# arkworks-rs/gemini

Hardware: AMD Instinct MI355X
Metric: BLS12-381 G1 MSM throughput (higher is better)
Workload: dtype u32x12 Montgomery Fq (381-bit integer), u32x8 Fr; 1 GPU; 2^20 G1 MSM per GPU (BASELINE configs[1]: 2^20 G1 MSM on one MI355X); pairs_per_gpu=1048576

## Files before the change

gemini_amd/csrc/msm.hip:

```cpp
#include <algorithm>
#include <atomic>
#include <chrono>
#include <condition_variable>
#include <cstdlib>
#include <cstring>
#include <functional>
#include <sched.h>
#include <cstdio>
#include <thread>
#include <vector>

#include "ctx.hpp"
#include "g1.cuh"
#include "host_field.hpp"

namespace gm {

constexpr uint32_t KEY_INV = 0xffffffffu;
constexpr int XYZZ_BYTES = 192;
constexpr int AFF_BYTES = 96;

struct DigitIter {
  uint32_t s[8];
  uint32_t carry;
// ... 556 lines not shown
  }
}

struct FlatGeom {
  int c, W;
  int glv;
  uint32_t B;
  uint32_t K[8];
};
template <bool SCATTER>
__global__ __launch_bounds__(256) void k_digits_flat(const uint32_t* __restrict__ scalars, uint32_t n, int mont, FlatGeom fg,
                                                     uint32_t* __restrict__ counts_or_cursor, uint64_t* __restrict__ entries,
                                                     uint32_t* __restrict__ err) {
  const uint32_t i = blockIdx.x * blockDim.x + threadIdx.x;
  const int half = (int)blockIdx.y >= fg.W ? 1 : 0;
  const int w = (int)blockIdx.y - half * fg.W;
  const bool active = i < n;
  uint32_t key = KEY_INV;
  bool neg = false;
  if (active) {
    Fr v = fp_load<FrParams>(scalars + 8 * (size_t)i);
    if (mont) v = fp_from_mont<FrParams>(v);
    if (!SCATTER && blockIdx.y == 0 && (v.l[7] >> 31)) atomicOr(err, 1u);
    bool hneg = false;
#ifdef GM_EXPERIMENTS
    if (fg.glv) {
      const GlvHalves h = glv_split(v.l);
      hneg = h.neg[half];
#pragma unroll
      for (int l = 0; l < 8; l++) v.l[l] = l < 4 ? h.m[half][l] : 0u;
    }
#endif
    uint32_t t[9];
    uint32_t carry = 0;
#pragma unroll
    for (int l = 0; l < 8; l++) {
      uint32_t cy;
      t[l] = __builtin_addc(v.l[l], fg.K[l], carry, &cy);
      carry = cy;
    }
    t[8] = carry;
    const uint32_t bit = (uint32_t)(fg.c * w), lo = bit >> 5, sh = bit & 31u;
    uint64_t two = 0;
#pragma unroll
    for (int l = 0; l < 9; l++) {
      if ((uint32_t)l == lo) two |= (uint64_t)t[l];
      if ((uint32_t)l == lo + 1) two |= (uint64_t)t[l] << 32;
    }
    uint32_t u = (uint32_t)(two >> sh);
    int32_t d;
    if (w == fg.W - 1) {
      d = (int32_t)min(u, fg.B);
    } else {
      u &= (1u << fg.c) - 1u;
      d = (int32_t)u - (int32_t)(1u << (fg.c - 1));
    }
    if (d != 0) {
      key = (uint32_t)w * fg.B + ((uint32_t)(d < 0 ? -d : d) - 1u);
      neg = (d < 0) != hneg;
    }
  }
  const uint32_t pos = wave_atomic_inc(counts_or_cursor, key);
  if (SCATTER && key != KEY_INV)
    entries[pos] = ((uint64_t)key << 32) | ((uint64_t)(neg ? 1u : 0u) << 31) | (uint64_t)(i | ((uint32_t)half << ENTRY_HALF_SHIFT));
}

struct MultiGeom {
  int c, W, levels, step;
  uint32_t B;
  uint32_t K[8];
  uint32_t start[MULTI_MAX_LEVELS + 1];
  const uint32_t* scal[MULTI_MAX_LEVELS];
  long long base0[MULTI_MAX_LEVELS];
};
template <bool SCATTER>
__global__ __launch_bounds__(256) void k_digits_multi(MultiGeom mg, int mont, uint32_t* __restrict__ counts_or_cursor, uint64_t* __restrict__ entries,
                                                      uint32_t* __restrict__ err) {
  const uint32_t i = blockIdx.x * blockDim.x + threadIdx.x;
  const int w = (int)blockIdx.y;
  const bool active = i < mg.start[mg.levels];
  uint32_t key = KEY_INV, idx = 0;
  bool neg = false;
  if (active) {
    int l = 0;
    while (l + 1 < mg.levels && i >= mg.start[l + 1]) l++;
    const uint32_t il = i - mg.start[l];
    Fr v = fp_load<FrParams>(mg.scal[l] + 8 * (size_t)il);
    if (mont) v = fp_from_mont<FrParams>(v);
    if (!SCATTER && blockIdx.y == 0 && (v.l[7] >> 31)) atomicOr(err, 1u);
    uint32_t t[9];
    uint32_t carry = 0;
#pragma unroll
    for (int q = 0; q < 8; q++) {
      uint32_t cy;
      t[q] = __builtin_addc(v.l[q], mg.K[q], carry, &cy);
      carry = cy;
    }
    t[8] = carry;
    const uint32_t bit = (uint32_t)(mg.c * w), lo = bit >> 5, sh = bit & 31u;
    uint64_t two = 0;
#pragma unroll
    for (int q = 0; q < 9; q++) {
      if ((uint32_t)q == lo) two |= (uint64_t)t[q];
      if ((uint32_t)q == lo + 1) two |= (uint64_t)t[q] << 32;
    }
    uint32_t u = (uint32_t)(two >> sh);
    int32_t d;
    if (w == mg.W - 1) {
      d = (int32_t)min(u, mg.B);
    } else {
      u &= (1u << mg.c) - 1u;
      d = (int32_t)u - (int32_t)(1u << (mg.c - 1));
    }
    if (d != 0) {
      key = (uint32_t)(l * mg.W + w) * mg.B + ((uint32_t)(d < 0 ? -d : d) - 1u);
      neg = d < 0;
      idx = (uint32_t)(mg.base0[l] + (long long)mg.step * (long long)il);
    }
  }
  const uint32_t pos = wave_atomic_inc(counts_or_cursor, key);
  if (SCATTER && key != KEY_INV) entries[pos] = ((uint64_t)key << 32) | ((uint64_t)(neg ? 1u : 0u) << 31) | (uint64_t)idx;
}


__global__ __launch_bounds__(1024) void k_scan_small(const uint32_t* __restrict__ counts, uint32_t m, uint32_t* __restrict__ offsets,
                                                     uint32_t* __restrict__ cursor) {
  __shared__ uint32_t part[1024];
  const uint32_t tid = threadIdx.x;
  const uint32_t per = (m + 1023u) / 1024u;
  const uint32_t lo = min(tid * per, m), hi = min(lo + per, m);
  uint32_t s = 0;
  for (uint32_t k = lo; k < hi; k++) s += counts[k];
  part[tid] = s;
  __syncthreads();
  for (uint32_t d = 1; d < 1024; d <<= 1) {
    const uint32_t x = tid >= d ? part[tid - d] : 0;
    __syncthreads();
    part[tid] += x;
    __syncthreads();
  }
  uint32_t run = part[tid] - s;
  for (uint32_t k = lo; k < hi; k++) {
    const uint32_t c = counts[k];
    offsets[k] = run;
    cursor[k] = run;
    run += c;
  }
  if (tid == 1023) offsets[m] = part[1023];
}

#ifdef GM_ACC0_CYCLES
__device__ unsigned long long gm_acc0_dbg[4];
#endif
template <int WAVES>
__global__ __launch_bounds__(256) __attribute__((amdgpu_waves_per_eu(WAVES, WAVES))) void k_acc0(const uint64_t* __restrict__ entries,
                                              const uint32_t* __restrict__ total_ptr,
                                              const uint8_t* __restrict__ bases, long long first, long long step,
                                              long long tab_stride, uint32_t L, uint32_t* __restrict__ pk,
                                              uint8_t* __restrict__ pp, uint8_t* __restrict__ buckets, const uint8_t* __restrict__ phi,
                                              unsigned long long* __restrict__ clk) {
  __shared__ uint64_t ebuf[8][256];
  const uint32_t t = blockIdx.x * blockDim.x + threadIdx.x;
  const uint64_t clk_c0 = clock64(), clk_w0 = wall_clock64();
  const uint64_t total = *total_ptr;
  const uint64_t start = (uint64_t)t * L;
  uint32_t head_key = KEY_INV, tail_key = KEY_INV;
#ifdef GM_ACC0_CYCLES
  const uint64_t dbg_c0 = clock64(), dbg_w0 = wall_clock64();
#endif
  if (start < total) {
    const uint64_t end = min(start + (uint64_t)L, total);
    Acc30 acc;
    acc30_zero(acc);
    uint32_t cur = KEY_INV;
    bool first_run = true;
    for (uint64_t i = start; i < end; i++) {
      const uint32_t k8 = (uint32_t)(i - start) & 7u;
      if (k8 == 0) {
        const uint4* src = reinterpret_cast<const uint4*>(entries + i);
#pragma unroll
        for (int q = 0; q < 4; q++) {
          const uint4 v = src[q];
          ebuf[2 * q][threadIdx.x] = ((uint64_t)v.y << 32) | v.x;
          ebuf[2 * q + 1][threadIdx.x] = ((uint64_t)v.w << 32) | v.z;
        }
      }
      const uint64_t e = ebuf[k8][threadIdx.x];
      long long idx;
      if (tab_stride) {
        const uint32_t lo = (uint32_t)e & 0x7fffffffu;
        idx = (long long)(lo >> ENTRY_W_SHIFT) * tab_stride + first + step * (long long)(lo & ((1u << ENTRY_W_SHIFT) - 1u));
      } else {
        idx = first + step * (long long)(e & 0x3fffffffull);
      }
      const uint8_t* src = (phi != nullptr && ((e >> ENTRY_HALF_SHIFT) & 1ull)) ? phi : bases;
      const gm_u4v* bp = reinterpret_cast<const gm_u4v*>(src + (size_t)idx * AFF_BYTES);
      const gm_u4v x0 = bp[0], x1 = bp[1], x2 = bp[2], y0 = bp[3], y1 = bp[4], y2 = bp[5];
      const uint32_t key = (uint32_t)(e >> 32);
      if (key != cur) {
        if (cur != KEY_INV) {
          if (first_run) {
            head_key = cur;
            acc30_store(pp + (size_t)(2 * (size_t)t) * XYZZ30_BYTES, acc);
            first_run = false;
          } else {
            acc30_store(buckets + (size_t)cur * XYZZ30_BYTES, acc);
          }
        }
        cur = key;
        acc30_set_identity(acc);
      }
      const uint32_t nz = x0.x | x0.y | x0.z | x0.w | x1.x | x1.y | x1.z | x1.w | x2.x | x2.y | x2.z | x2.w | y0.x | y0.y | y0.z | y0.w |
                          y1.x | y1.y | y1.z | y1.w | y2.x | y2.y | y2.z | y2.w;
      if (nz == 0) continue;
      const uint32_t neg = (uint32_t)(e >> 31) & 1u;
      (void)g1_madd30_asm(acc, x0, x1, x2, y0, y1, y2, neg);
    }
    if (first_run) {
      head_key = cur;
      acc30_store(pp + (size_t)(2 * (size_t)t) * XYZZ30_BYTES, acc);
    } else {
      tail_key = cur;
      acc30_store(pp + (size_t)(2 * (size_t)t + 1) * XYZZ30_BYTES, acc);
    }
  }
  pk[2 * (size_t)t] = head_key;
  pk[2 * (size_t)t + 1] = tail_key;
  if (t == 0 && clk != nullptr) {
    clk[0] = (unsigned long long)(clock64() - clk_c0);
    clk[1] = (unsigned long long)(wall_clock64() - clk_w0);
  }
#ifdef GM_ACC0_CYCLES
  if ((threadIdx.x & 63) == 0) {
    atomicAdd(&gm_acc0_dbg[0], (unsigned long long)(clock64() - dbg_c0));
    atomicAdd(&gm_acc0_dbg[1], (unsigned long long)(wall_clock64() - dbg_w0));
    atomicAdd(&gm_acc0_dbg[2], 1ull);
  }
#endif
}

template <int WAVES>
__global__ __launch_bounds__(256) __attribute__((amdgpu_waves_per_eu(WAVES, WAVES))) void k_acc0_pf(const uint64_t* __restrict__ entries,
                                              const uint32_t* __restrict__ total_ptr,
                                              const uint8_t* __restrict__ bases, long long first, long long step,
                                              long long tab_stride, uint32_t L, uint32_t* __restrict__ pk,
                                              uint8_t* __restrict__ pp, uint8_t* __restrict__ buckets, const uint8_t* __restrict__ phi,
                                              unsigned long long* __restrict__ clk) {
  __shared__ uint64_t ebuf[8][256];
  const uint32_t t = blockIdx.x * blockDim.x + threadIdx.x;
  const uint64_t clk_c0 = clock64(), clk_w0 = wall_clock64();
  const uint64_t total = *total_ptr;
  const uint64_t start = (uint64_t)t * L;
  uint32_t head_key = KEY_INV, tail_key = KEY_INV;
  if (start < total) {
    const uint64_t end = min(start + (uint64_t)L, total);
    Acc30 acc;
    acc30_zero(acc);
    uint32_t cur = KEY_INV;
    bool first_run = true;
    auto entry_at = [&](uint64_t i) {
      const uint32_t k8 = (uint32_t)(i - start) & 7u;
      if (k8 == 0) {
        const uint4* src = reinterpret_cast<const uint4*>(entries + i);
#pragma unroll
        for (int q = 0; q < 4; q++) {
          const uint4 v = src[q];
          ebuf[2 * q][threadIdx.x] = ((uint64_t)v.y << 32) | v.x;
          ebuf[2 * q + 1][threadIdx.x] = ((uint64_t)v.w << 32) | v.z;
        }
      }
      return ebuf[k8][threadIdx.x];
    };
    auto base_of = [&](uint64_t e) {
      long long idx;
      if (tab_stride) {
        const uint32_t lo = (uint32_t)e & 0x7fffffffu;
        idx = (long long)(lo >> ENTRY_W_SHIFT) * tab_stride + first + step * (long long)(lo & ((1u << ENTRY_W_SHIFT) - 1u));
      } else {
        idx = first + step * (long long)(e & 0x3fffffffull);
      }
      const uint8_t* src = (phi != nullptr && ((e >> ENTRY_HALF_SHIFT) & 1ull)) ? phi : bases;
      return reinterpret_cast<const gm_u4v*>(src + (size_t)idx * AFF_BYTES);
    };
    uint64_t e = entry_at(start);
    const gm_u4v* bp = base_of(e);
    gm_u4v x0 = bp[0], x1 = bp[1], x2 = bp[2], y0 = bp[3], y1 = bp[4], y2 = bp[5];
    for (uint64_t i = start; i < end; i++) {
      uint64_t en = 0;
      gm_u4v n0 = x0, n1 = x1, n2 = x2, n3 = y0, n4 = y1, n5 = y2;
      if (i + 1 < end) {
        en = entry_at(i + 1);
        const gm_u4v* np = base_of(en);
        asm volatile(
            "global_load_dwordx4 %0, %6, off\n\t"
            "global_load_dwordx4 %1, %6, off offset:16\n\t"
            "global_load_dwordx4 %2, %6, off offset:32\n\t"
            "global_load_dwordx4 %3, %6, off offset:48\n\t"
            "global_load_dwordx4 %4, %6, off offset:64\n\t"
            "global_load_dwordx4 %5, %6, off offset:80"
            : "=&v"(n0), "=&v"(n1), "=&v"(n2), "=&v"(n3), "=&v"(n4), "=&v"(n5)
            : "v"(np));
      }
      const uint32_t key = (uint32_t)(e >> 32);
      if (key != cur) {
        if (cur != KEY_INV) {
          if (first_run) {
            head_key = cur;
            acc30_store(pp + (size_t)(2 * (size_t)t) * XYZZ30_BYTES, acc);
            first_run = false;
          } else {
            acc30_store(buckets + (size_t)cur * XYZZ30_BYTES, acc);
          }
        }
        cur = key;
        acc30_set_identity(acc);
      }
      const uint32_t nz = x0.x | x0.y | x0.z | x0.w | x1.x | x1.y | x1.z | x1.w | x2.x | x2.y | x2.z | x2.w | y0.x | y0.y | y0.z | y0.w |
                          y1.x | y1.y | y1.z | y1.w | y2.x | y2.y | y2.z | y2.w;
      if (nz != 0) {
        const uint32_t neg = (uint32_t)(e >> 31) & 1u;
        (void)g1_madd30_asm(acc, x0, x1, x2, y0, y1, y2, neg);
      }
      asm volatile("s_waitcnt vmcnt(0)" : "+v"(n0), "+v"(n1), "+v"(n2), "+v"(n3), "+v"(n4), "+v"(n5));
      e = en;
      x0 = n0; x1 = n1; x2 = n2; y0 = n3; y1 = n4; y2 = n5;
    }
    if (first_run) {
      head_key = cur;
      acc30_store(pp + (size_t)(2 * (size_t)t) * XYZZ30_BYTES, acc);
    } else {
      tail_key = cur;
      acc30_store(pp + (size_t)(2 * (size_t)t + 1) * XYZZ30_BYTES, acc);
    }
  }
  pk[2 * (size_t)t] = head_key;
  pk[2 * (size_t)t + 1] = tail_key;
  if (t == 0 && clk != nullptr) {
    clk[0] = (unsigned long long)(clock64() - clk_c0);
    clk[1] = (unsigned long long)(wall_clock64() - clk_w0);
  }
}

#ifdef GM_EXPERIMENTS
#include "msm_levels.inc"
#endif

__global__ __launch_bounds__(64) void k_merge(const uint32_t* __restrict__ keys_in, const uint8_t* __restrict__ pts_in,
                                              uint32_t E, uint32_t* __restrict__ keys_out,
                                              uint8_t* __restrict__ pts_out, uint8_t* __restrict__ buckets,
                                              int final_level) {
  __shared__ __attribute__((aligned(16))) uint8_t lds[128 * XYZZ30_BYTES];
  const int lane = threadIdx.x;
  const uint32_t wave = blockIdx.x;
  const uint32_t s0 = wave * 128u + 2u * lane;
  uint32_t hk = s0 < E ? keys_in[s0] : KEY_INV;
  uint32_t tk = s0 + 1 < E ? keys_in[s0 + 1] : KEY_INV;
  uint32_t hs = 2 * lane, ts = 2 * lane + 1;
  auto copy_rec = [](void* dst, const void* src) {
    const gm_u4v* s = reinterpret_cast<const gm_u4v*>(src);
    gm_u4v* d = reinterpret_cast<gm_u4v*>(dst);
#pragma unroll
    for (int i = 0; i < 13; i++) d[i] = s[i];
  };
  auto add_slots = [&](uint32_t dst_slot, uint32_t src_slot, Acc30& a) {
    Acc30 o;
    acc30_load(a, lds + dst_slot * XYZZ30_BYTES);
    acc30_load(o, lds + src_slot * XYZZ30_BYTES);
    acc30_add(a, o);
  };
  if (hk != KEY_INV) copy_rec(lds + hs * XYZZ30_BYTES, pts_in + (size_t)s0 * XYZZ30_BYTES);
  if (tk != KEY_INV) copy_rec(lds + ts * XYZZ30_BYTES, pts_in + ((size_t)s0 + 1) * XYZZ30_BYTES);
  if (hk == KEY_INV && tk != KEY_INV) {
    hk = tk;
    hs = ts;
    tk = KEY_INV;
  }
  __syncthreads();
  if (hk != KEY_INV && hk == tk) {
    Acc30 a;
    add_slots(hs, ts, a);
    acc30_store(lds + hs * XYZZ30_BYTES, a);
    tk = KEY_INV;
  }
  __syncthreads();

  {
    const uint32_t nhk = __shfl_down(hk, 1), nhs = __shfl_down(hs, 1), ntk = __shfl_down(tk, 1);
    const uint32_t ptk = __shfl_up(tk, 1);
    const bool give = lane < 63 && tk != KEY_INV && ntk != KEY_INV && nhk == tk;
    const bool taken = lane > 0 && tk != KEY_INV && ptk != KEY_INV && ptk == hk;
    if (__any(give)) {
      if (give) {
        Acc30 a;
        add_slots(ts, nhs, a);
        acc30_store(buckets + (size_t)tk * XYZZ30_BYTES, a);
      }
    }
    __syncthreads();
    if (taken) {
      hk = tk; hs = ts; tk = KEY_INV;
    }
    if (give) {
      if (taken) { hk = KEY_INV; } else { tk = KEY_INV; }
    }
  }

  for (int d = 1; d < 64; d <<= 1) {
    const uint32_t bhk = __shfl_down(hk, d), bhs = __shfl_down(hs, d);
    const uint32_t btk = __shfl_down(tk, d), bts = __shfl_down(ts, d);
    const bool act = (lane & (2 * d - 1)) == 0;
    bool do_add = false;
    uint32_t add_dst = 0, add_src = 0;
    uint32_t f1k = KEY_INV, f1s = 0, f2k = KEY_INV, f2s = 0;
    if (act && bhk != KEY_INV) {
      if (hk == KEY_INV) {
        hk = bhk; hs = bhs; tk = btk; ts = bts;
      } else {
        const bool a_two = tk != KEY_INV, b_two = btk != KEY_INV;
        const uint32_t alk = a_two ? tk : hk, als = a_two ? ts : hs;
        if (alk == bhk) {
          do_add = true; add_dst = als; add_src = bhs;
          if (b_two) {
            if (a_two) { f1k = alk; f1s = als; }
            tk = btk; ts = bts;
          }
        } else {
          if (a_two) { f1k = tk; f1s = ts; }
          if (b_two) { f2k = bhk; f2s = bhs; tk = btk; ts = bts; }
          else { tk = bhk; ts = bhs; }
        }
      }
    }
    if (__any(do_add)) {
      if (do_add) {
        Acc30 a;
        add_slots(add_dst, add_src, a);
        acc30_store(lds + add_dst * XYZZ30_BYTES, a);
      }
    }
    if (f1k != KEY_INV) copy_rec(buckets + (size_t)f1k * XYZZ30_BYTES, lds + f1s * XYZZ30_BYTES);
    if (f2k != KEY_INV) copy_rec(buckets + (size_t)f2k * XYZZ30_BYTES, lds + f2s * XYZZ30_BYTES);
    __syncthreads();
  }
  if (lane == 0) {
    if (final_level) {
      if (hk != KEY_INV) copy_rec(buckets + (size_t)hk * XYZZ30_BYTES, lds + hs * XYZZ30_BYTES);
      if (tk != KEY_INV) copy_rec(buckets + (size_t)tk * XYZZ30_BYTES, lds + ts * XYZZ30_BYTES);
    } else {
      keys_out[2 * (size_t)wave] = hk;
      keys_out[2 * (size_t)wave + 1] = tk;
      if (hk != KEY_INV) copy_rec(pts_out + (size_t)(2 * (size_t)wave) * XYZZ30_BYTES, lds + hs * XYZZ30_BYTES);
      if (tk != KEY_INV) copy_rec(pts_out + (size_t)(2 * (size_t)wave + 1) * XYZZ30_BYTES, lds + ts * XYZZ30_BYTES);
    }
  }
}

enum { GS_STRIDED = 0, GS_PLANE = 1 };
struct GroupSumArgs {
  const uint8_t* in;
  uint8_t* out;
  int mode;
  uint32_t n_out;
  uint32_t per_win;
  uint32_t win_stride;
  uint32_t n_lo, s_hi, s_lo, s_e, len;
  uint32_t nb;
  uint32_t lpo_shift;
  int out_canonical;
  const uint32_t* in_cnt;
};
struct GroupSumJobs {
  GroupSumArgs j[3];
  uint32_t blk_end[3];
  const uint32_t* err_src;
  uint32_t* err_dst;
  const unsigned long long* clk_src;
};

__global__ __launch_bounds__(256) void k_group_sum(GroupSumJobs J) {
  if (J.err_dst && blockIdx.x == 0 && threadIdx.x == 0) {
    *J.err_dst = *J.err_src;
    if (J.clk_src) {
      unsigned long long* d = reinterpret_cast<unsigned long long*>(J.err_dst + 2);
      d[0] = J.clk_src[0];
      d[1] = J.clk_src[1];
    }
  }
  const int job = blockIdx.x < J.blk_end[0] ? 0 : (blockIdx.x < J.blk_end[1] ? 1 : 2);
  const GroupSumArgs& a = J.j[job];
  const uint32_t blk0 = job == 0 ? 0u : J.blk_end[job - 1];
  const uint8_t* __restrict__ in = a.in;
  uint8_t* __restrict__ out = a.out;
  const uint32_t gt = (blockIdx.x - blk0) * blockDim.x + threadIdx.x;
  const uint32_t lpo = 1u << a.lpo_shift;
  const uint32_t o = gt >> a.lpo_shift, q = gt & (lpo - 1u);
  Acc30 acc;
  acc30_zero(acc);
  const uint32_t* __restrict__ in_cnt = a.in_cnt;
  auto filled = [&](size_t slot) { return in_cnt == nullptr || in_cnt[slot] != 0u; };
  auto add_rec = [&](size_t slot) {
    if (!filled(slot)) return;
    Acc30 v;
    acc30_load(v, in + slot * XYZZ30_BYTES);
    acc30_add(acc, v);
  };
  auto load_first = [&](size_t slot) {
    if (filled(slot)) acc30_load(acc, in + slot * XYZZ30_BYTES);
  };
  if (o < a.n_out) {
    const uint32_t w = o / a.per_win, r = o % a.per_win;
    const size_t base = (size_t)w * a.win_stride;
    if (a.mode == GS_STRIDED) {
      const size_t b0 = base + (size_t)(r / a.n_lo) * a.s_hi + (size_t)(r % a.n_lo) * a.s_lo;
      if (q < a.len) load_first(b0 + (size_t)q * a.s_e);
      for (uint32_t e = q + lpo; e < a.len; e += lpo) add_rec(b0 + (size_t)e * a.s_e);
    } else {
// ... 764 lines not shown
  LevelGeom lg{};
  if (multi_block) {
    lg.levels = multi->levels;
    lg.step = (int)step;
    uint32_t at = 0;
    for (int l = 0; l < multi->levels; l++) {
      lg.start[l] = at;
      lg.scal[l] = reinterpret_cast<const uint32_t*>(multi->scalars[l]);
      lg.base0[l] = (long long)multi->start[l];
      at += (uint32_t)multi->n[l];
    }
    lg.start[multi->levels] = at;
  }
  if (multi && !multi_block) {
    MultiGeom mg{};
    mg.c = c;
    mg.W = W;
    mg.levels = multi->levels;
    mg.step = (int)step;
    mg.B = B;
    for (int j = 0; j + 1 < W; j++) {
      const int b = c * j + c - 1;
      if (b < 256) mg.K[b >> 5] |= 1u << (b & 31);
    }
    uint32_t at = 0;
    for (int l = 0; l < multi->levels; l++) {
      mg.start[l] = at;
      mg.scal[l] = reinterpret_cast<const uint32_t*>(multi->scalars[l]);
      mg.base0[l] = (long long)multi->start[l];
      at += (uint32_t)multi->n[l];
    }
    mg.start[multi->levels] = at;
    GM_CHECK(N <= ((uint64_t)1 << 21) && nbuckets <= ((size_t)1 << 18), GM_EINVAL, "msm: fused calls too large for the flat sort (%llu entries, %zu buckets)",
             (unsigned long long)N, nbuckets);
    const dim3 grid((uint32_t)((n + 255) / 256), (uint32_t)W);
    pf.begin(part, PROF_DIGITS, st);
    hipLaunchKernelGGL(k_digits_multi<false>, grid, dim3(256), 0, st, mg, mont, ws.counts.as<uint32_t>(), (uint64_t*)nullptr, d_err);
    hipLaunchKernelGGL(k_scan_small, dim3(1), dim3(1024), 0, st, ws.counts.as<uint32_t>(), (uint32_t)nbuckets, ws.offsets.as<uint32_t>(),
                       ws.cursor.as<uint32_t>());
    pf.end(part, PROF_DIGITS, st);
    pf.begin(part, PROF_SCATTER, st);
    hipLaunchKernelGGL(k_digits_multi<true>, grid, dim3(256), 0, st, mg, mont, ws.cursor.as<uint32_t>(), ws.entries.as<uint64_t>(), d_err);
    pf.end(part, PROF_SCATTER, st);
  } else if (sort_flat) {
    FlatGeom fg{};
    fg.c = c;
    fg.W = W;
    fg.glv = use_glv ? 1 : 0;
    fg.B = B;
    for (int j = 0; j + 1 < W; j++) {
      const int b = c * j + c - 1;
      if (b < 256) fg.K[b >> 5] |= 1u << (b & 31);
    }
    const dim3 grid((uint32_t)((n + 255) / 256), (uint32_t)(W * (use_glv ? 2 : 1)));
    pf.begin(part, PROF_DIGITS, st);
    hipLaunchKernelGGL(k_digits_flat<false>, grid, dim3(256), 0, st, sc, (uint32_t)n, mont, fg, ws.counts.as<uint32_t>(), (uint64_t*)nullptr, d_err);
    hipLaunchKernelGGL(k_scan_small, dim3(1), dim3(1024), 0, st, ws.counts.as<uint32_t>(), (uint32_t)nbuckets, ws.offsets.as<uint32_t>(),
                       ws.cursor.as<uint32_t>());
    pf.end(part, PROF_DIGITS, st);
    pf.begin(part, PROF_SCATTER, st);
    hipLaunchKernelGGL(k_digits_flat<true>, grid, dim3(256), 0, st, sc, (uint32_t)n, mont, fg, ws.cursor.as<uint32_t>(), ws.entries.as<uint64_t>(), d_err);
    pf.end(part, PROF_SCATTER, st);
  } else if (sort_atomic) {
    pf.begin(part, PROF_DIGITS, st);
    hipLaunchKernelGGL(k_msm_digits<false>, dim3(dblocks), dim3(256), 0, st, sc, (uint32_t)n, mont, c, W, B,
                       ws.counts.as<uint32_t>(), (uint64_t*)nullptr, d_err);
    pf.end(part, PROF_DIGITS, st);
    pf.begin(part, PROF_SCAN, st);
    run_scan();
    pf.end(part, PROF_SCAN, st);
    pf.begin(part, PROF_SCATTER, st);
    hipLaunchKernelGGL(k_msm_digits<true>, dim3(dblocks), dim3(256), 0, st, sc, (uint32_t)n, mont, c, W, B,
                       ws.cursor.as<uint32_t>(), ws.entries.as<uint64_t>(), d_err);
    pf.end(part, PROF_SCATTER, st);
  } else {
    SortGeom sg;
    sg.c = c;
    sg.W = W;
    sg.w_lo = use_table ? 0 : w_lo;
    sg.Wg = use_table ? W : Wg;
    sg.glv = use_glv ? 1 : 0;
    sg.B = B;
    sg.shared = use_table ? 1 : 0;
    sg.FB = std::min<uint32_t>((uint32_t)(c - 1), 10u);
    if (multi_block) sg.FB = std::min<uint32_t>((uint32_t)(c - 1), std::max<uint32_t>(sg.FB, 11u));
    while ((nbuckets >> sg.FB) > SORT_GMAX && (1u << sg.FB) < SORT_FMAX) sg.FB++;
    sg.G = (uint32_t)(nbuckets >> sg.FB);
    GM_CHECK(sg.G <= SORT_GMAX, GM_EINVAL, "msm: %u coarse sort bins exceed %u (window %d too wide for this sort)", sg.G, SORT_GMAX, c);
    if ((rc = ws.tmp_entries.ensure(N * 8))) return rc;
    if ((rc = ws.sortmeta.ensure((size_t)(3 * (sg.G + 1)) * 4))) return rc;
    uint32_t* gcount = ws.counts.as<uint32_t>() + nbuckets + 2;
    uint32_t* goff = ws.sortmeta.as<uint32_t>();
    uint32_t* gcursor = goff + (sg.G + 1);
    uint32_t* blkoff = gcursor + (sg.G + 1);
    const uint32_t b1 = (uint32_t)((n + SORT_TS - 1) / SORT_TS);
    const uint32_t b2 = (uint32_t)(N / SORT_CH + sg.G + 1);
    pf.begin(part, PROF_DIGITS, st);
    hipLaunchKernelGGL(k_sort1<false>, dim3(b1), dim3(256), 0, st, sc, (uint32_t)n, mont, sg, lg, gcount, (uint64_t*)nullptr, d_err);
    hipLaunchKernelGGL(k_sort1_scan, dim3(1), dim3(1024), 0, st, gcount, sg.G, goff, gcursor, blkoff);
    const size_t stage1_lds = (size_t)SORT_TS * sg.Wg * (use_glv ? 2 : 1) * 8 + (size_t)3 * sg.G * 4 + 1024 * 4;
    static const bool sort1_staged_env = !(getenv("GM_MSM_SORT1") && !strcmp(getenv("GM_MSM_SORT1"), "direct"));
    if (sort1_staged_env && sg.Wg * (use_glv ? 2 : 1) <= SORT1_STAGE_WMAX && stage1_lds <= 160 * 1024) {
      static bool attr_set = false;
      if (!attr_set) {
        GM_HIP(hipFuncSetAttribute(reinterpret_cast<const void*>(k_sort1_staged), hipFuncAttributeMaxDynamicSharedMemorySize, 160 * 1024));
        attr_set = true;
      }
      hipLaunchKernelGGL(k_sort1_staged, dim3(b1), dim3(1024), stage1_lds, st, sc, (uint32_t)n, mont, sg, lg, gcursor, ws.tmp_entries.as<uint64_t>());
    } else {
      hipLaunchKernelGGL(k_sort1<true>, dim3(b1), dim3(256), 0, st, sc, (uint32_t)n, mont, sg, lg, gcursor, ws.tmp_entries.as<uint64_t>(), d_err);
    }
    pf.end(part, PROF_DIGITS, st);
    pf.begin(part, PROF_SCATTER, st);
    hipLaunchKernelGGL(k_sort2<false>, dim3(b2), dim3(256), 0, st, ws.tmp_entries.as<uint64_t>(), goff, blkoff, sg,
                       ws.counts.as<uint32_t>(), (uint64_t*)nullptr);
    run_scan();
    static const bool sort_staged = !(getenv("GM_MSM_SORT2") && !strcmp(getenv("GM_MSM_SORT2"), "direct"));
    if (sort_staged && (1u << sg.FB) <= SORT_STAGE_FMAX)
      hipLaunchKernelGGL(k_sort2_staged, dim3(b2), dim3(1024), 0, st, ws.tmp_entries.as<uint64_t>(), goff, blkoff, sg,
                         ws.cursor.as<uint32_t>(), ws.entries.as<uint64_t>());
    else
      hipLaunchKernelGGL(k_sort2<true>, dim3(b2), dim3(256), 0, st, ws.tmp_entries.as<uint64_t>(), goff, blkoff, sg,
                         ws.cursor.as<uint32_t>(), ws.entries.as<uint64_t>());
    pf.end(part, PROF_SCATTER, st);
  }
  const uint64_t* acc_entries = ws.entries.as<uint64_t>();
  const uint32_t* acc_total = ws.offsets.as<uint32_t>() + nbuckets;
  const uint8_t* acc_bases = d_bases;
  long long acc_first = (long long)first, acc_step = multi ? 1ll : (long long)step, acc_tab = tab_stride;
#ifdef GM_EXPERIMENTS
#define GM_MSM_LEVELS_HOST 1
#include "msm_levels.inc"
#undef GM_MSM_LEVELS_HOST
#else
  GM_CHECK(levels == 0, GM_EINVAL, "msm: affine tree levels are an experiment of round 2; rebuild with -DGM_EXPERIMENTS (DESIGN.md section 8)");
#endif
  if (!ws.have_done_ev) {
    for (int e = 0; e < MSM_SLOTS; e++) GM_HIP(hipEventCreateWithFlags(&ws.done_ev[e], hipEventDisableTiming));
    GM_HIP(hipEventCreateWithFlags(&ws.sort_ev, hipEventDisableTiming));
    GM_HIP(hipEventCreateWithFlags(&ws.acc_ev, hipEventDisableTiming));
    ws.have_done_ev = true;
  }
  if (sts.acc != st) {
    GM_HIP(hipEventRecord(ws.sort_ev, st));
    GM_HIP(hipStreamWaitEvent(sts.acc, ws.sort_ev, 0));
  }
  st = sts.acc;
  pf.begin(part, PROF_ACC0, st);
  static const size_t acc0_lds_pad = getenv("GM_ACC0_LDS_PAD") ? (size_t)strtoull(getenv("GM_ACC0_LDS_PAD"), nullptr, 10) : 0;
  if ((rc = ws.clk.ensure(16))) return rc;
  unsigned long long* acc_clk = ws.clk.as<unsigned long long>();
  static const int acc0_pf_env = getenv("GM_ACC0_PREFETCH") ? atoi(getenv("GM_ACC0_PREFETCH")) : -1;
  const bool acc0_pf = acc0_pf_env >= 0 ? acc0_pf_env != 0 : use_table;
  if (acc0_pf)
    hipLaunchKernelGGL(k_acc0_pf<2>, dim3((uint32_t)(T0pad / 256)), dim3(256), 0, st, acc_entries, acc_total, acc_bases, acc_first, acc_step,
                       acc_tab, L, ws.pk[0].as<uint32_t>(), ws.pp[0].as<uint8_t>(), ws.buckets.as<uint8_t>(), use_glv ? bases->phi : (const uint8_t*)nullptr, acc_clk);
  else if (acc0_waves == 2)
    hipLaunchKernelGGL(k_acc0<2>, dim3((uint32_t)(T0pad / 256)), dim3(256), acc0_lds_pad, st, acc_entries, acc_total, acc_bases, acc_first, acc_step,
                       acc_tab, L, ws.pk[0].as<uint32_t>(), ws.pp[0].as<uint8_t>(), ws.buckets.as<uint8_t>(), use_glv ? bases->phi : (const uint8_t*)nullptr, acc_clk);
  else
    hipLaunchKernelGGL(k_acc0<3>, dim3((uint32_t)(T0pad / 256)), dim3(256), 0, st, acc_entries, acc_total, acc_bases, acc_first, acc_step,
                       acc_tab, L, ws.pk[0].as<uint32_t>(), ws.pp[0].as<uint8_t>(), ws.buckets.as<uint8_t>(), use_glv ? bases->phi : (const uint8_t*)nullptr, acc_clk);
  pf.end(part, PROF_ACC0, st);
  if (sts.tail != st) {
    GM_HIP(hipEventRecord(ws.acc_ev, st));
    GM_HIP(hipStreamWaitEvent(sts.tail, ws.acc_ev, 0));
  }
  st = sts.tail;
  pf.begin(part, PROF_MERGE, st);
  {
    uint64_t E = E1;
    int src = 0;
    for (;;) {
      uint32_t waves = (uint32_t)((E + 127) / 128);
      int final_level = waves == 1;
      hipLaunchKernelGGL(k_merge, dim3(waves), dim3(64), 0, st, ws.pk[src].as<uint32_t>(), ws.pp[src].as<uint8_t>(),
                         (uint32_t)E, ws.pk[src ^ 1].as<uint32_t>(), ws.pp[src ^ 1].as<uint8_t>(),
                         ws.buckets.as<uint8_t>(), final_level);
      if (final_level) break;
      E = 2ull * waves;
      src ^= 1;
    }
  }

  pf.end(part, PROF_MERGE, st);
  pf.begin(part, PROF_REDUCE, st);
  const uint32_t nbits = (uint32_t)(c - 1);
  uint32_t wf[3] = {0, 0, 0};
  int m;
  static const int fields_env = getenv("GM_MSM_FIELDS") ? atoi(getenv("GM_MSM_FIELDS")) : 0;
  if (nbits <= 7) {
    m = 1;
    wf[0] = nbits;
  } else if (nbits <= 14 || (fields_env == 2 && nbits <= 16)) {
    m = 2;
    wf[0] = nbits / 2;
    wf[1] = nbits - wf[0];
  } else {
    m = 3;
    static const bool odd_low = !(getenv("GM_MSM_ODD_BIT") && !strcmp(getenv("GM_MSM_ODD_BIT"), "high"));
    wf[0] = odd_low ? (nbits + 2) / 3 : nbits / 3;
    wf[1] = (nbits - wf[0]) / 2;
    wf[2] = nbits - wf[0] - wf[1];
  }
  static const int lpo_env = getenv("GM_MSM_LPO_LOG") ? atoi(getenv("GM_MSM_LPO_LOG")) : 0;
  const int lpo_target_log = lpo_env ? lpo_env : (nbuckets >= ((size_t)1 << 21) ? 18 : 17);
  uint32_t lpo_jobs = 1;
  auto lpo_for = [&](uint32_t len, uint32_t n_out) {
    uint32_t s = 0;
    while (s < 5 && (1u << s) < len && ((uint64_t)n_out << s) * lpo_jobs < (1ull << lpo_target_log)) s++;
    return s;
  };
  const uint8_t* bucket_in = ws.buckets.as<uint8_t>();
  const uint32_t* bucket_cnt = bucket_counts_valid ? ws.counts.as<uint32_t>() : nullptr;
  auto strided = [&](const uint8_t* in, uint8_t* out, uint32_t win_in, uint32_t n_hi, uint32_t n_lo, uint32_t s_hi, uint32_t s_lo,
                     uint32_t s_e, uint32_t len) {
    GroupSumArgs g{};
    g.in = in; g.out = out; g.mode = GS_STRIDED; g.in_cnt = in == bucket_in ? bucket_cnt : nullptr;
    g.per_win = n_hi * n_lo; g.n_out = (uint32_t)Wb * g.per_win; g.win_stride = win_in;
    g.n_lo = n_lo; g.s_hi = s_hi; g.s_lo = s_lo; g.s_e = s_e; g.len = len; g.lpo_shift = lpo_for(len, g.n_out);
    return g;
  };
  auto plane = [&](const uint8_t* in, uint8_t* out, uint32_t nb) {
    GroupSumArgs g{};
    g.in = in; g.out = out; g.mode = GS_PLANE; g.out_canonical = 1;
    g.in_cnt = in == bucket_in ? bucket_cnt : nullptr;
    g.per_win = nb + 1; g.n_out = (uint32_t)Wb * g.per_win; g.win_stride = 1u << nb; g.nb = nb;
    g.lpo_shift = lpo_for(nb ? (1u << (nb - 1)) : 1u, g.n_out);
    return g;
  };
  uint8_t* planes = nullptr;
  size_t plane_count = 0;
  auto launch = [&](std::initializer_list<GroupSumArgs> jobs, bool last = false) {
    GroupSumJobs J{};
    if (last) {
      J.err_src = d_err;
      J.err_dst = reinterpret_cast<uint32_t*>(planes + plane_count * XYZZ_BYTES);
      J.clk_src = ws.clk.as<unsigned long long>();
    }
    uint32_t tot = 0;
    int k = 0;
    for (const GroupSumArgs& g : jobs) {
      J.j[k] = g;
      tot += (uint32_t)((((uint64_t)g.n_out << g.lpo_shift) + 255) / 256);
      J.blk_end[k] = tot;
      k++;
    }
    for (; k < 3; k++) J.blk_end[k] = tot;
    hipLaunchKernelGGL(k_group_sum, dim3(tot), dim3(256), 0, st, J);
  };
  size_t plane_off[3];
  for (int k = 0; k < m; k++) {
    plane_off[k] = plane_count;
    plane_count += (size_t)Wb * (wf[k] + 1);
  }
  const size_t plane_bytes = plane_count * XYZZ_BYTES + 24;
  if (ws.host_planes_cap[slot] < plane_bytes) {
    if (ws.host_planes[slot]) (void)hipHostFree(ws.host_planes[slot]);
    ws.host_planes[slot] = nullptr;
    ws.host_planes_cap[slot] = 0;
    GM_HIP(hipHostMalloc((void**)&ws.host_planes[slot], plane_bytes, hipHostMallocDefault));
    ws.host_planes_cap[slot] = plane_bytes;
  }
  const bool zc = (C->zero_copy & 2) != 0;
  if (zc) {
    planes = reinterpret_cast<uint8_t*>(ws.host_planes[slot]);
  } else {
    if ((rc = ws.planes.ensure(plane_count * XYZZ_BYTES + 64))) return rc;
    planes = ws.planes.as<uint8_t>();
  }
  const uint8_t* X = ws.buckets.as<uint8_t>();
  const uint32_t n0 = 1u << wf[0], n1 = 1u << wf[1], n2 = 1u << wf[2];
  if (m == 1) {
    lpo_jobs = 1;
    launch({plane(X, planes, wf[0])}, true);
  } else if (m == 2) {
    if ((rc = ws.rows.ensure((size_t)Wb * (n0 + n1) * XYZZ30_BYTES))) return rc;
    uint8_t* Y0 = ws.rows.as<uint8_t>();
    uint8_t* Y1 = Y0 + (size_t)Wb * n0 * XYZZ30_BYTES;
    lpo_jobs = 2;
    launch({strided(X, Y1, B, 1, n1, 0, n0, 1, n0), strided(X, Y0, B, 1, n0, 0, 1, n0, n1)});
    launch({plane(Y0, planes + plane_off[0] * XYZZ_BYTES, wf[0]), plane(Y1, planes + plane_off[1] * XYZZ_BYTES, wf[1])}, true);
  } else {
    if ((rc = ws.rows.ensure((size_t)Wb * ((size_t)n2 * n1 + (size_t)n2 * n0) * XYZZ30_BYTES))) return rc;
    if ((rc = ws.cols.ensure((size_t)Wb * (n0 + n1 + n2) * XYZZ30_BYTES))) return rc;
    uint8_t* A = ws.rows.as<uint8_t>();
    uint8_t* Bm = A + (size_t)Wb * n2 * n1 * XYZZ30_BYTES;
    uint8_t* Y0 = ws.cols.as<uint8_t>();
    uint8_t* Y1 = Y0 + (size_t)Wb * n0 * XYZZ30_BYTES;
    uint8_t* Y2 = Y1 + (size_t)Wb * n1 * XYZZ30_BYTES;
    lpo_jobs = 2;
    launch({strided(X, A, B, n2, n1, n1 * n0, n0, 1, n0), strided(X, Bm, B, n2, n0, n1 * n0, 1, n0, n1)});
    lpo_jobs = 3;
    launch({strided(A, Y2, n2 * n1, 1, n2, 0, n1, 1, n1), strided(A, Y1, n2 * n1, 1, n1, 0, 1, n1, n2),
            strided(Bm, Y0, n2 * n0, 1, n0, 0, 1, n0, n2)});
    launch({plane(Y0, planes + plane_off[0] * XYZZ_BYTES, wf[0]), plane(Y1, planes + plane_off[1] * XYZZ_BYTES, wf[1]),
            plane(Y2, planes + plane_off[2] * XYZZ_BYTES, wf[2])}, true);
  }
  pf.end(part, PROF_REDUCE, st);
  GM_HIP(hipGetLastError());
  if (!zc) GM_HIP(hipMemcpyAsync(ws.host_planes[slot], planes, plane_bytes, hipMemcpyDeviceToHost, st));
  GM_HIP(hipEventRecord(ws.done_ev[slot], st));
  P->Wb = Wb;
  P->multi_levels = multi ? multi->levels : 0;
  P->multi_W = multi ? (use_table ? 1 : W) : 0;
  P->plane_count = plane_count;
  P->c = c;
  P->m = m;
  P->nbits = nbits;
  for (int k = 0; k < 3; k++) {
    P->wf[k] = wf[k];
    P->plane_off[k] = k < m ? plane_off[k] : 0;
  }
  return GM_OK;
}
// ... 641 lines not shown
```

Baseline: 347.7 Mscalar/s.

## Hand off head runs between neighbor lanes via LDS mailbox and fast-path merge

In the acc0 bucket-accumulation kernel, each thread publishes its first (head) run into an LDS mailbox. A neighbour lane whose tail run has the same key absorbs that accumulator directly and writes the bucket itself, so fewer partial records go through the merge tree. The change also merges the prefetch and plain acc0 kernels into one template, and adds a ballot-based fast path to k_merge that copies records straight out when no keys in a wave clash. The cost is extra dynamic LDS (about 53KB per block), wave fences, and an extra global read of each thread's last entry key.

Measured after the change: 348.9 Mscalar/s, median of 4. No clear change (+0.3%).

```diff
diff --git a/gemini_amd/csrc/msm.hip b/gemini_amd/csrc/msm.hip
--- a/gemini_amd/csrc/msm.hip
+++ b/gemini_amd/csrc/msm.hip
@@ -732,7 +732,26 @@
 #ifdef GM_ACC0_CYCLES
 __device__ unsigned long long gm_acc0_dbg[4];
 #endif
-template <int WAVES>
+constexpr size_t ACC0_MBOX_BYTES = 256 * (size_t)XYZZ30_BYTES + 256 * 4 + 256 * 4;
+GM_DEV void acc0_wave_fence() {
+  __builtin_amdgcn_fence(__ATOMIC_SEQ_CST, "wavefront");
+  __builtin_amdgcn_wave_barrier();
+}
+GM_DEV void acc0_mbox_store(gm_u4v* m, const Acc30& A) {
+  m[0 * 256] = A.a0.lo; m[1 * 256] = A.a0.hi; m[2 * 256] = A.a1.lo; m[3 * 256] = A.a1.hi; m[4 * 256] = A.a2.lo; m[5 * 256] = A.a2.hi;
+  m[6 * 256] = A.a3.lo; m[7 * 256] = A.a3.hi; m[8 * 256] = A.a4.lo; m[9 * 256] = A.a4.hi; m[10 * 256] = A.a5.lo; m[11 * 256] = A.a5.hi;
+  m[12 * 256] = A.a6;
+}
+GM_DEV void acc0_mbox_load(Acc30& A, const gm_u4v* m) {
+  A.a0 = __builtin_shufflevector(m[0 * 256], m[1 * 256], 0, 1, 2, 3, 4, 5, 6, 7);
+  A.a1 = __builtin_shufflevector(m[2 * 256], m[3 * 256], 0, 1, 2, 3, 4, 5, 6, 7);
+  A.a2 = __builtin_shufflevector(m[4 * 256], m[5 * 256], 0, 1, 2, 3, 4, 5, 6, 7);
+  A.a3 = __builtin_shufflevector(m[6 * 256], m[7 * 256], 0, 1, 2, 3, 4, 5, 6, 7);
+  A.a4 = __builtin_shufflevector(m[8 * 256], m[9 * 256], 0, 1, 2, 3, 4, 5, 6, 7);
+  A.a5 = __builtin_shufflevector(m[10 * 256], m[11 * 256], 0, 1, 2, 3, 4, 5, 6, 7);
+  A.a6 = m[12 * 256];
+}
+template <int WAVES, bool PF, bool HANDOFF>
 __global__ __launch_bounds__(256) __attribute__((amdgpu_waves_per_eu(WAVES, WAVES))) void k_acc0(const uint64_t* __restrict__ entries,
                                               const uint32_t* __restrict__ total_ptr,
                                               const uint8_t* __restrict__ bases, long long first, long long step,
@@ -740,11 +759,22 @@
                                               uint8_t* __restrict__ pp, uint8_t* __restrict__ buckets, const uint8_t* __restrict__ phi,
                                               unsigned long long* __restrict__ clk) {
   __shared__ uint64_t ebuf[8][256];
+  extern __shared__ __attribute__((aligned(16))) uint8_t acc0_mbox[];
+  gm_u4v* const mb_rec = reinterpret_cast<gm_u4v*>(acc0_mbox);
+  uint32_t* const mb_key = reinterpret_cast<uint32_t*>(acc0_mbox + 256 * (size_t)XYZZ30_BYTES);
+  uint32_t* const mb_taken = mb_key + 256;
+  const uint32_t tid = threadIdx.x;
   const uint32_t t = blockIdx.x * blockDim.x + threadIdx.x;
   const uint64_t clk_c0 = clock64(), clk_w0 = wall_clock64();
   const uint64_t total = *total_ptr;
   const uint64_t start = (uint64_t)t * L;
   uint32_t head_key = KEY_INV, tail_key = KEY_INV;
+  bool published = false;
+  if constexpr (HANDOFF) {
+    mb_key[tid] = KEY_INV;
+    mb_taken[tid] = 0u;
+    acc0_wave_fence();
+  }
 #ifdef GM_ACC0_CYCLES
   const uint64_t dbg_c0 = clock64(), dbg_w0 = wall_clock64();
 #endif
@@ -753,91 +783,9 @@
     Acc30 acc;
     acc30_zero(acc);
     uint32_t cur = KEY_INV;
-    bool first_run = true;
-    for (uint64_t i = start; i < end; i++) {
-      const uint32_t k8 = (uint32_t)(i - start) & 7u;
-      if (k8 == 0) {
-        const uint4* src = reinterpret_cast<const uint4*>(entries + i);
-#pragma unroll
-        for (int q = 0; q < 4; q++) {
-          const uint4 v = src[q];
-          ebuf[2 * q][threadIdx.x] = ((uint64_t)v.y << 32) | v.x;
-          ebuf[2 * q + 1][threadIdx.x] = ((uint64_t)v.w << 32) | v.z;
-        }
-      }
-      const uint64_t e = ebuf[k8][threadIdx.x];
-      long long idx;
-      if (tab_stride) {
-        const uint32_t lo = (uint32_t)e & 0x7fffffffu;
-        idx = (long long)(lo >> ENTRY_W_SHIFT) * tab_stride + first + step * (long long)(lo & ((1u << ENTRY_W_SHIFT) - 1u));
-      } else {
-        idx = first + step * (long long)(e & 0x3fffffffull);
-      }
-      const uint8_t* src = (phi != nullptr && ((e >> ENTRY_HALF_SHIFT) & 1ull)) ? phi : bases;
-      const gm_u4v* bp = reinterpret_cast<const gm_u4v*>(src + (size_t)idx * AFF_BYTES);
-      const gm_u4v x0 = bp[0], x1 = bp[1], x2 = bp[2], y0 = bp[3], y1 = bp[4], y2 = bp[5];
-      const uint32_t key = (uint32_t)(e >> 32);
-      if (key != cur) {
-        if (cur != KEY_INV) {
-          if (first_run) {
-            head_key = cur;
-            acc30_store(pp + (size_t)(2 * (size_t)t) * XYZZ30_BYTES, acc);
-            first_run = false;
-          } else {
-            acc30_store(buckets + (size_t)cur * XYZZ30_BYTES, acc);
-          }
-        }
-        cur = key;
-        acc30_set_identity(acc);
-      }
-      const uint32_t nz = x0.x | x0.y | x0.z | x0.w | x1.x | x1.y | x1.z | x1.w | x2.x | x2.y | x2.z | x2.w | y0.x | y0.y | y0.z | y0.w |
-                          y1.x | y1.y | y1.z | y1.w | y2.x | y2.y | y2.z | y2.w;
-      if (nz == 0) continue;
-      const uint32_t neg = (uint32_t)(e >> 31) & 1u;
-      (void)g1_madd30_asm(acc, x0, x1, x2, y0, y1, y2, neg);
-    }
-    if (first_run) {
-      head_key = cur;
-      acc30_store(pp + (size_t)(2 * (size_t)t) * XYZZ30_BYTES, acc);
-    } else {
-      tail_key = cur;
-      acc30_store(pp + (size_t)(2 * (size_t)t + 1) * XYZZ30_BYTES, acc);
-    }
-  }
-  pk[2 * (size_t)t] = head_key;
-  pk[2 * (size_t)t + 1] = tail_key;
-  if (t == 0 && clk != nullptr) {
-    clk[0] = (unsigned long long)(clock64() - clk_c0);
-    clk[1] = (unsigned long long)(wall_clock64() - clk_w0);
-  }
-#ifdef GM_ACC0_CYCLES
-  if ((threadIdx.x & 63) == 0) {
-    atomicAdd(&gm_acc0_dbg[0], (unsigned long long)(clock64() - dbg_c0));
-    atomicAdd(&gm_acc0_dbg[1], (unsigned long long)(wall_clock64() - dbg_w0));
-    atomicAdd(&gm_acc0_dbg[2], 1ull);
-  }
-#endif
-}
-
-template <int WAVES>
-__global__ __launch_bounds__(256) __attribute__((amdgpu_waves_per_eu(WAVES, WAVES))) void k_acc0_pf(const uint64_t* __restrict__ entries,
-                                              const uint32_t* __restrict__ total_ptr,
-                                              const uint8_t* __restrict__ bases, long long first, long long step,
-                                              long long tab_stride, uint32_t L, uint32_t* __restrict__ pk,
-                                              uint8_t* __restrict__ pp, uint8_t* __restrict__ buckets, const uint8_t* __restrict__ phi,
-                                              unsigned long long* __restrict__ clk) {
-  __shared__ uint64_t ebuf[8][256];
-  const uint32_t t = blockIdx.x * blockDim.x + threadIdx.x;
-  const uint64_t clk_c0 = clock64(), clk_w0 = wall_clock64();
-  const uint64_t total = *total_ptr;
-  const uint64_t start = (uint64_t)t * L;
-  uint32_t head_key = KEY_INV, tail_key = KEY_INV;
-  if (start < total) {
-    const uint64_t end = min(start + (uint64_t)L, total);
-    Acc30 acc;
-    acc30_zero(acc);
-    uint32_t cur = KEY_INV;
-    bool first_run = true;
+    bool first_run = true, took = false;
+    uint32_t last_key = KEY_INV;
+    if constexpr (HANDOFF) last_key = (uint32_t)(entries[end - 1] >> 32);
     auto entry_at = [&](uint64_t i) {
       const uint32_t k8 = (uint32_t)(i - start) & 7u;
       if (k8 == 0) {
@@ -862,38 +810,65 @@
       const uint8_t* src = (phi != nullptr && ((e >> ENTRY_HALF_SHIFT) & 1ull)) ? phi : bases;
       return reinterpret_cast<const gm_u4v*>(src + (size_t)idx * AFF_BYTES);
     };
-    uint64_t e = entry_at(start);
-    const gm_u4v* bp = base_of(e);
-    gm_u4v x0 = bp[0], x1 = bp[1], x2 = bp[2], y0 = bp[3], y1 = bp[4], y2 = bp[5];
+    uint64_t e = 0;
+    gm_u4v x0, x1, x2, y0, y1, y2;
+    if constexpr (PF) {
+      e = entry_at(start);
+      const gm_u4v* bp = base_of(e);
+      x0 = bp[0]; x1 = bp[1]; x2 = bp[2]; y0 = bp[3]; y1 = bp[4]; y2 = bp[5];
+    }
     for (uint64_t i = start; i < end; i++) {
       uint64_t en = 0;
-      gm_u4v n0 = x0, n1 = x1, n2 = x2, n3 = y0, n4 = y1, n5 = y2;
-      if (i + 1 < end) {
-        en = entry_at(i + 1);
-        const gm_u4v* np = base_of(en);
-        asm volatile(
-            "global_load_dwordx4 %0, %6, off\n\t"
-            "global_load_dwordx4 %1, %6, off offset:16\n\t"
-            "global_load_dwordx4 %2, %6, off offset:32\n\t"
-            "global_load_dwordx4 %3, %6, off offset:48\n\t"
-            "global_load_dwordx4 %4, %6, off offset:64\n\t"
-            "global_load_dwordx4 %5, %6, off offset:80"
-            : "=&v"(n0), "=&v"(n1), "=&v"(n2), "=&v"(n3), "=&v"(n4), "=&v"(n5)
-            : "v"(np));
+      gm_u4v n0, n1, n2, n3, n4, n5;
+      if constexpr (PF) {
+        n0 = x0; n1 = x1; n2 = x2; n3 = y0; n4 = y1; n5 = y2;
+        if (i + 1 < end) {
+          en = entry_at(i + 1);
+          const gm_u4v* np = base_of(en);
+          asm volatile(
+              "global_load_dwordx4 %0, %6, off\n\t"
+              "global_load_dwordx4 %1, %6, off offset:16\n\t"
+              "global_load_dwordx4 %2, %6, off offset:32\n\t"
+              "global_load_dwordx4 %3, %6, off offset:48\n\t"
+              "global_load_dwordx4 %4, %6, off offset:64\n\t"
+              "global_load_dwordx4 %5, %6, off offset:80"
+              : "=&v"(n0), "=&v"(n1), "=&v"(n2), "=&v"(n3), "=&v"(n4), "=&v"(n5)
+              : "v"(np));
+        }
+      } else {
+        e = entry_at(i);
+        const gm_u4v* bp = base_of(e);
+        x0 = bp[0]; x1 = bp[1]; x2 = bp[2]; y0 = bp[3]; y1 = bp[4]; y2 = bp[5];
       }
       const uint32_t key = (uint32_t)(e >> 32);
       if (key != cur) {
         if (cur != KEY_INV) {
           if (first_run) {
             head_key = cur;
-            acc30_store(pp + (size_t)(2 * (size_t)t) * XYZZ30_BYTES, acc);
+            if constexpr (HANDOFF) {
+              acc0_mbox_store(mb_rec + tid, acc);
+              mb_key[tid] = cur;
+              published = true;
+            } else {
+              acc30_store(pp + (size_t)(2 * (size_t)t) * XYZZ30_BYTES, acc);
+            }
             first_run = false;
           } else {
             acc30_store(buckets + (size_t)cur * XYZZ30_BYTES, acc);
           }
         }
+        bool take = false;
+        if constexpr (HANDOFF) {
+          acc0_wave_fence();
+          take = cur != KEY_INV && key == last_key && (tid & 63u) != 63u && mb_key[tid + 1] == key;
+          if (take) {
+            acc0_mbox_load(acc, mb_rec + tid + 1);
+            mb_taken[tid + 1] = 1u;
+            took = true;
+          }
+        }
         cur = key;
-        acc30_set_identity(acc);
+        if (!take) acc30_set_identity(acc);
       }
       const uint32_t nz = x0.x | x0.y | x0.z | x0.w | x1.x | x1.y | x1.z | x1.w | x2.x | x2.y | x2.z | x2.w | y0.x | y0.y | y0.z | y0.w |
                           y1.x | y1.y | y1.z | y1.w | y2.x | y2.y | y2.z | y2.w;
@@ -901,16 +876,32 @@
         const uint32_t neg = (uint32_t)(e >> 31) & 1u;
         (void)g1_madd30_asm(acc, x0, x1, x2, y0, y1, y2, neg);
       }
-      asm volatile("s_waitcnt vmcnt(0)" : "+v"(n0), "+v"(n1), "+v"(n2), "+v"(n3), "+v"(n4), "+v"(n5));
-      e = en;
-      x0 = n0; x1 = n1; x2 = n2; y0 = n3; y1 = n4; y2 = n5;
+      if constexpr (PF) {
+        asm volatile("s_waitcnt vmcnt(0)" : "+v"(n0), "+v"(n1), "+v"(n2), "+v"(n3), "+v"(n4), "+v"(n5));
+        e = en;
+        x0 = n0; x1 = n1; x2 = n2; y0 = n3; y1 = n4; y2 = n5;
+      }
     }
     if (first_run) {
       head_key = cur;
       acc30_store(pp + (size_t)(2 * (size_t)t) * XYZZ30_BYTES, acc);
+    } else if (took) {
+      acc30_store(buckets + (size_t)cur * XYZZ30_BYTES, acc);
     } else {
       tail_key = cur;
       acc30_store(pp + (size_t)(2 * (size_t)t + 1) * XYZZ30_BYTES, acc);
+    }
+  }
+  if constexpr (HANDOFF) {
+    acc0_wave_fence();
+    if (published) {
+      if (mb_taken[tid]) {
+        head_key = KEY_INV;
+      } else {
+        gm_u4v* o = reinterpret_cast<gm_u4v*>(pp + (size_t)(2 * (size_t)t) * XYZZ30_BYTES);
+#pragma unroll
+        for (int q = 0; q < 13; q++) o[q] = mb_rec[q * 256 + tid];
+      }
     }
   }
   pk[2 * (size_t)t] = head_key;
@@ -919,6 +910,13 @@
     clk[0] = (unsigned long long)(clock64() - clk_c0);
     clk[1] = (unsigned long long)(wall_clock64() - clk_w0);
   }
+#ifdef GM_ACC0_CYCLES
+  if ((threadIdx.x & 63) == 0) {
+    atomicAdd(&gm_acc0_dbg[0], (unsigned long long)(clock64() - dbg_c0));
+    atomicAdd(&gm_acc0_dbg[1], (unsigned long long)(wall_clock64() - dbg_w0));
+    atomicAdd(&gm_acc0_dbg[2], 1ull);
+  }
+#endif
 }
 
 #ifdef GM_EXPERIMENTS
@@ -942,6 +940,32 @@
 #pragma unroll
     for (int i = 0; i < 13; i++) d[i] = s[i];
   };
+  {
+    const bool hv = hk != KEY_INV, tv = tk != KEY_INV;
+    const uint64_t mh = __ballot(hv), mt = __ballot(tv);
+    const int nrec = __popcll(mh) + __popcll(mt);
+    const uint64_t front = (mh | mt) & ((1ull << lane) - 1ull);
+    const uint32_t prev_key = __shfl(tv ? tk : hk, front ? 63 - __clzll((long long)front) : lane);
+    const bool clash = (hv && tv && hk == tk) || ((hv || tv) && front != 0 && prev_key == (hv ? hk : tk));
+    if (!__any(clash)) {
+      const uint32_t rank = (uint32_t)(__popcll(mh & ((1ull << lane) - 1ull)) + __popcll(mt & ((1ull << lane) - 1ull)));
+      auto emit = [&](uint32_t r, uint32_t key, uint32_t slot) {
+        const uint8_t* src = pts_in + (size_t)slot * XYZZ30_BYTES;
+        if (final_level || (r != 0 && r + 1 != (uint32_t)nrec)) {
+          copy_rec(buckets + (size_t)key * XYZZ30_BYTES, src);
+        } else {
+          const size_t o = 2 * (size_t)wave + (r != 0 ? 1 : 0);
+          keys_out[o] = key;
+          copy_rec(pts_out + o * XYZZ30_BYTES, src);
+        }
+      };
+      if (hv) emit(rank, hk, s0);
+      if (tv) emit(rank + (hv ? 1u : 0u), tk, s0 + 1);
+      if (lane == 0 && !final_level)
+        for (int r = nrec; r < 2; r++) keys_out[2 * (size_t)wave + r] = KEY_INV;
+      return;
+    }
+  }
   auto add_slots = [&](uint32_t dst_slot, uint32_t src_slot, Acc30& a) {
     Acc30 o;
     acc30_load(a, lds + dst_slot * XYZZ30_BYTES);
@@ -2012,15 +2036,30 @@
   unsigned long long* acc_clk = ws.clk.as<unsigned long long>();
   static const int acc0_pf_env = getenv("GM_ACC0_PREFETCH") ? atoi(getenv("GM_ACC0_PREFETCH")) : -1;
   const bool acc0_pf = acc0_pf_env >= 0 ? acc0_pf_env != 0 : use_table;
-  if (acc0_pf)
-    hipLaunchKernelGGL(k_acc0_pf<2>, dim3((uint32_t)(T0pad / 256)), dim3(256), 0, st, acc_entries, acc_total, acc_bases, acc_first, acc_step,
+  static const bool acc0_handoff_env = !(getenv("GM_ACC0_HANDOFF") && atoi(getenv("GM_ACC0_HANDOFF")) == 0);
+  const bool acc0_handoff = acc0_handoff_env && (acc0_pf || acc0_waves == 2);
+  auto launch_acc0 = [&](auto kernel, size_t dyn_lds) {
+    hipLaunchKernelGGL(kernel, dim3((uint32_t)(T0pad / 256)), dim3(256), dyn_lds, st, acc_entries, acc_total, acc_bases, acc_first, acc_step,
                        acc_tab, L, ws.pk[0].as<uint32_t>(), ws.pp[0].as<uint8_t>(), ws.buckets.as<uint8_t>(), use_glv ? bases->phi : (const uint8_t*)nullptr, acc_clk);
-  else if (acc0_waves == 2)
-    hipLaunchKernelGGL(k_acc0<2>, dim3((uint32_t)(T0pad / 256)), dim3(256), acc0_lds_pad, st, acc_entries, acc_total, acc_bases, acc_first, acc_step,
-                       acc_tab, L, ws.pk[0].as<uint32_t>(), ws.pp[0].as<uint8_t>(), ws.buckets.as<uint8_t>(), use_glv ? bases->phi : (const uint8_t*)nullptr, acc_clk);
-  else
-    hipLaunchKernelGGL(k_acc0<3>, dim3((uint32_t)(T0pad / 256)), dim3(256), 0, st, acc_entries, acc_total, acc_bases, acc_first, acc_step,
-                       acc_tab, L, ws.pk[0].as<uint32_t>(), ws.pp[0].as<uint8_t>(), ws.buckets.as<uint8_t>(), use_glv ? bases->phi : (const uint8_t*)nullptr, acc_clk);
+  };
+  if (acc0_handoff) {
+    static bool attr_set[64] = {};
+    int dev = 0;
+    GM_HIP(hipGetDevice(&dev));
+    if (dev >= 0 && dev < 64 && !attr_set[dev]) {
+      GM_HIP(hipFuncSetAttribute(reinterpret_cast<const void*>(k_acc0<2, false, true>), hipFuncAttributeMaxDynamicSharedMemorySize, 128 * 1024));
+      GM_HIP(hipFuncSetAttribute(reinterpret_cast<const void*>(k_acc0<2, true, true>), hipFuncAttributeMaxDynamicSharedMemorySize, 128 * 1024));
+      attr_set[dev] = true;
+    }
+    if (acc0_pf) launch_acc0(k_acc0<2, true, true>, ACC0_MBOX_BYTES);
+    else launch_acc0(k_acc0<2, false, true>, ACC0_MBOX_BYTES + acc0_lds_pad);
+  } else if (acc0_pf) {
+    launch_acc0(k_acc0<2, true, false>, 0);
+  } else if (acc0_waves == 2) {
+    launch_acc0(k_acc0<2, false, false>, acc0_lds_pad);
+  } else {
+    launch_acc0(k_acc0<3, false, false>, 0);
+  }
   pf.end(part, PROF_ACC0, st);
   if (sts.tail != st) {
     GM_HIP(hipEventRecord(ws.acc_ev, st));
```
